# GuidoManni/BodySLAM

Hardware: AMD Instinct MI355X
Metric: frames/sec depth+pose+back-proj, 640x480 seq (higher is better)
Workload: dtype f16

## Files before the change

bodyslam_amd/csrc/upconv_fused.hip:

```cpp
#include "common.h"

namespace bs {

namespace ucf {
constexpr int C = 128, CO = 32, TW = 16, TH = 16, LW = 11, LH = 11, NR = LW * LH;
constexpr int TAB = 2048;
constexpr int PLANE = NR * 128;
constexpr int WROWS = 3 * CO;
constexpr int WPLANE = WROWS * 128;
constexpr int YSTRIDE = 400;
constexpr int YBYTES = NR * YSTRIDE;
template <int MODE> constexpr int a_planes() { return 2 + MODE; }
template <int MODE> constexpr int lds_bytes() { return TAB + a_planes<MODE>() * PLANE + a_planes<MODE>() * WPLANE + YBYTES; }
}

struct UpconvFusedArgs {
    const void* x;
    const void* w;
    const float* bias;
    void* out;
    int B, Hin, Win, Hout, Wout;
    float sy, sx;
    int relu, ntx, nty, ntiles;
    int sa0, sb0, sa1, sb1;
};

template <typename T, int SPLIT, int MODE>
__global__ __launch_bounds__(512) void upconv_fused_kernel(const UpconvFusedArgs p) {
    using namespace ucf;
    typedef typename T16<T>::v8 v8;
    typedef int i32x4_ __attribute__((ext_vector_type(4)));
    typedef int i32x8_ __attribute__((ext_vector_type(8)));
    typedef float f32x2 __attribute__((ext_vector_type(2)));
    constexpr int NPL = a_planes<MODE>();
    constexpr bool FULL = MODE == 2;
    constexpr int ROWB = MODE == 0 ? 2 * C : 4 * C;
    constexpr int OFF_A = TAB, OFF_W = OFF_A + NPL * PLANE, OFF_Y = OFF_W + NPL * WPLANE;
    extern __shared__ __attribute__((aligned(16))) char smem[];
    const int tid = threadIdx.x, lane = tid & 63;
    const int wave = __builtin_amdgcn_readfirstlane(tid >> 6);
    const int frow = lane & 15, fq = lane >> 4;
    const int Hin = p.Hin, Win = p.Win, Hout = p.Hout, Wout = p.Wout;

    auto lo_idx = [&](int r, float s, int n) {
        int i0 = (int)(s * (float)r);
        return i0 > n - 1 ? n - 1 : i0;
    };
    struct Win_ { int b, ty0, tx0, wy0, wx0, LWc, LHc; };
    auto window = [&](int tile) {
        Win_ w;
        const int txi = tile % p.ntx, t2 = tile / p.ntx;
        w.tx0 = txi * TW;
        w.ty0 = (t2 % p.nty) * TH;
        w.b = t2 / p.nty;
        const int rmin = w.ty0 > 0 ? w.ty0 - 1 : 0, rmax = w.ty0 + TH < Hout ? w.ty0 + TH : Hout - 1;
        const int cmin = w.tx0 > 0 ? w.tx0 - 1 : 0, cmax = w.tx0 + TW < Wout ? w.tx0 + TW : Wout - 1;
        w.wy0 = lo_idx(rmin, p.sy, Hin);
        w.wx0 = lo_idx(cmin, p.sx, Win);
        int wy1 = lo_idx(rmax, p.sy, Hin), wx1 = lo_idx(cmax, p.sx, Win);
        wy1 += wy1 < Hin - 1 ? 1 : 0;
        wx1 += wx1 < Win - 1 ? 1 : 0;
        w.LWc = wx1 - w.wx0 + 1;
        w.LHc = wy1 - w.wy0 + 1;
        return w;
    };
    const int r8 = lane >> 3, chunk = (lane & 7) ^ r8;
    auto issue_window = [&](const Win_& w) {
        const int nv = w.LWc * w.LHc;
        const char* xb = reinterpret_cast<const char*>(p.x) + ((int64_t)w.b * Hin * Win) * ROWB;
#pragma unroll
        for (int h = 0; h < 2; ++h) {
            const int rg = wave + 8 * h, row = rg * 8 + r8;
            if (row < NR) {
                const int rw = row < nv ? row : nv - 1;
                const int ly = rw / w.LWc, lx = rw - ly * w.LWc;
                const char* px = xb + ((int64_t)(w.wy0 + ly) * Win + (w.wx0 + lx)) * ROWB + chunk * 16;
#pragma unroll
                for (int pl = 0; pl < NPL; ++pl)
                    glds16(px + pl * 128, smem + OFF_A + pl * PLANE + rg * 1024);
            }
        }
    };
    auto issue_weights = [&](int ky) {
        const char* wb = reinterpret_cast<const char*>(p.w) + (int64_t)(ky * WROWS) * ROWB + chunk * 16;
#pragma unroll
        for (int h = 0; h < 2; ++h) {
            const int rg = wave + 8 * h;
            if (rg < WROWS / 8) {
                const char* pw = wb + (int64_t)(rg * 8 + r8) * ROWB;
#pragma unroll
                for (int pl = 0; pl < NPL; ++pl)
                    glds16(pw + pl * 128, smem + OFF_W + pl * WPLANE + rg * 1024);
            }
        }
    };

    const int g = tid & 7, X = (tid >> 3) & 15, seg = tid >> 7;
    const f32x4 bias4 = *reinterpret_cast<const f32x4*>(p.bias + 4 * g);
    const int sca0 = p.sa0 * 0x01010101, scb0 = p.sb0 * 0x01010101, sca1 = p.sa1 * 0x01010101, scb1 = p.sb1 * 0x01010101;
    const int sw = frow & 7;
    const int koff0 = (fq ^ sw) << 4, koff1 = ((4 + fq) ^ sw) << 4;

    int tile = blockIdx.x;
    if (tile >= p.ntiles) return;
    Win_ cur = window(tile);
    issue_window(cur);
    issue_weights(0);
    for (int it = 0; tile < p.ntiles; tile += gridDim.x, ++it) {
        const int next = tile + gridDim.x;
        i32x4_* tabs = reinterpret_cast<i32x4_*>(smem + (it & 1) * (TAB / 2));
        if (tid < TH + 2 + TW + 2) {
            const bool isrow = tid < TH + 2;
            const int r = isrow ? cur.ty0 - 1 + tid : cur.tx0 - 1 + (tid - (TH + 2));
            const int nout = isrow ? Hout : Wout, nin = isrow ? Hin : Win, w0 = isrow ? cur.wy0 : cur.wx0;
            const float s = isrow ? p.sy : p.sx;
            const int unit = isrow ? cur.LWc * YSTRIDE : YSTRIDE;
            i32x4_ e = {0, 0, 0, 0};
            if (r >= 0 && r < nout) {
                const float f = s * (float)r;
                int i0 = (int)f;
                i0 = i0 > nin - 1 ? nin - 1 : i0;
                const int i1 = i0 + (i0 < nin - 1 ? 1 : 0);
                const float l = f - (float)i0, h = 1.0f - l;
                e = i32x4_{(i0 - w0) * unit, (i1 - w0) * unit, __float_as_int(h), __float_as_int(l)};
            }
            tabs[tid] = e;
        }
        const int mg = wave >> 1, ng = wave & 1;
        v8 af[2][4];
        i32x8_ a8h[2], a8l[2];
        f32x4 acc[4];
#pragma unroll
        for (int yy = 0; yy < 4; ++yy) acc[yy] = bias4;
        i32x4_ ctab[3];
#pragma unroll
        for (int ky = 0; ky < 3; ++ky) {
            if (ky == 1 && next < p.ntiles && !(p.relu & 32)) asm volatile("s_waitcnt vmcnt(%0)" ::"n"(2 * NPL) : "memory");
            else asm volatile("s_waitcnt vmcnt(0)" ::: "memory");
            __syncthreads();
            auto ld8 = [&](const char* base) {
                const i32x4_ lo = *reinterpret_cast<const i32x4_*>(base + koff0);
                const i32x4_ hi = *reinterpret_cast<const i32x4_*>(base + koff1);
                return __builtin_shufflevector(lo, hi, 0, 1, 2, 3, 4, 5, 6, 7);
            };
            if (ky == 0) {
#pragma unroll
                for (int i = 0; i < 2; ++i) {
                    const char* ar = smem + OFF_A + (mg * 32 + i * 16 + frow) * 128;
#pragma unroll
                    for (int kk = 0; kk < 4; ++kk) af[i][kk] = *reinterpret_cast<const v8*>(ar + (kk >> 1) * PLANE + ((kk & 1) ? koff1 : koff0));
                    if constexpr (MODE >= 1) a8h[i] = ld8(ar + 2 * PLANE);
                    if constexpr (FULL) a8l[i] = ld8(ar + 3 * PLANE);
                }
#pragma unroll
                for (int kx = 0; kx < 3; ++kx) ctab[kx] = tabs[TH + 2 + X + kx];
            }
            if (!(p.relu & 8)) {
#pragma unroll
                for (int j = 0; j < 3; ++j) {
                    const char* wr = smem + OFF_W + (ng * 48 + j * 16 + frow) * 128;
                    v8 wf[4];
#pragma unroll
                    for (int kk = 0; kk < 4; ++kk) wf[kk] = *reinterpret_cast<const v8*>(wr + (kk >> 1) * WPLANE + ((kk & 1) ? koff1 : koff0));
                    i32x8_ w8l, w8h;
                    if constexpr (MODE >= 1) w8l = ld8(wr + 2 * WPLANE);
                    if constexpr (FULL) w8h = ld8(wr + 3 * WPLANE);
#pragma unroll
                    for (int i = 0; i < 2; ++i) {
                        f32x4 c = {0.f, 0.f, 0.f, 0.f};
#pragma unroll
                        for (int kk = 0; kk < 4; ++kk) c = T16<T>::mfma16(wf[kk], af[i][kk], c);
                        if constexpr (MODE >= 1) c = __builtin_amdgcn_mfma_scale_f32_16x16x128_f8f6f4(w8l, a8h[i], c, 0, 0, 0, scb0, 0, sca0);
                        if constexpr (FULL) c = __builtin_amdgcn_mfma_scale_f32_16x16x128_f8f6f4(w8h, a8l[i], c, 0, 0, 0, scb1, 0, sca1);
                        const int m = mg * 32 + i * 16 + frow;
                        if (m < NR) *reinterpret_cast<f32x4*>(smem + OFF_Y + m * YSTRIDE + (ng * 48 + j * 16) * 4 + fq * 16) = c;
                    }
                }
            }
            __syncthreads();
            if (ky < 2) {
                if (!(p.relu & 2)) issue_weights(ky + 1);
                if (ky == 0 && next < p.ntiles && !(p.relu & 32)) {
                    const Win_ nw = window(next);
                    issue_window(nw);
                }
            } else if (next < p.ntiles) {
                if (!(p.relu & 2)) issue_weights(0);
            }
            if (!(p.relu & 4)) {
                const char* yb = smem + OFF_Y + g * 16;
                auto rowsum = [&](int roff) {
                    f32x2 u01 = {0.f, 0.f}, u23 = {0.f, 0.f};
#pragma unroll
                    for (int kx = 0; kx < 3; ++kx) {
                        const char* q = yb + roff + kx * (CO * 4);
                        const f32x4 q0 = *reinterpret_cast<const f32x4*>(q + ctab[kx][0]);
                        const f32x4 q1 = *reinterpret_cast<const f32x4*>(q + ctab[kx][1]);
                        const float hx = __int_as_float(ctab[kx][2]), lx = __int_as_float(ctab[kx][3]);
                        const f32x2 h2 = {hx, hx}, l2 = {lx, lx};
                        u01 = __builtin_elementwise_fma(h2, f32x2{q0[0], q0[1]}, u01);
                        u23 = __builtin_elementwise_fma(h2, f32x2{q0[2], q0[3]}, u23);
                        u01 = __builtin_elementwise_fma(l2, f32x2{q1[0], q1[1]}, u01);
                        u23 = __builtin_elementwise_fma(l2, f32x2{q1[2], q1[3]}, u23);
                    }
                    return f32x4{u01[0], u01[1], u23[0], u23[1]};
                };
                int have0 = -1, have1 = -1;
                f32x4 U0 = {0.f, 0.f, 0.f, 0.f}, U1 = U0;
#pragma unroll
                for (int yy = 0; yy < 4; ++yy) {
                    const i32x4_ ry = tabs[4 * seg + yy + ky];
                    const int o0 = __builtin_amdgcn_readfirstlane(ry[0]), o1 = __builtin_amdgcn_readfirstlane(ry[1]);
                    if (o0 != have0) {
                        U0 = (o0 == have1) ? U1 : rowsum(o0);
                        have0 = o0;
                    }
                    if (o1 != have1) {
                        U1 = (o1 == have0) ? U0 : rowsum(o1);
                        have1 = o1;
                    }
                    const float hy = __int_as_float(ry[2]), ly = __int_as_float(ry[3]);
                    const f32x2 h2 = {hy, hy}, l2 = {ly, ly};
                    f32x2 a01 = {acc[yy][0], acc[yy][1]}, a23 = {acc[yy][2], acc[yy][3]};
                    a01 = __builtin_elementwise_fma(h2, f32x2{U0[0], U0[1]}, a01);
                    a23 = __builtin_elementwise_fma(h2, f32x2{U0[2], U0[3]}, a23);
                    a01 = __builtin_elementwise_fma(l2, f32x2{U1[0], U1[1]}, a01);
                    a23 = __builtin_elementwise_fma(l2, f32x2{U1[2], U1[3]}, a23);
                    acc[yy] = f32x4{a01[0], a01[1], a23[0], a23[1]};
                }
            }
        }
        const int ox = cur.tx0 + X;
#pragma unroll
        for (int yy = 0; yy < 4; ++yy) {
            const int oy = cur.ty0 + 4 * seg + yy;
            if (ox >= Wout || oy >= Hout || (p.relu & 16)) continue;
            f32x4 a = acc[yy];
            if (p.relu & 1) {
#pragma unroll
                for (int e = 0; e < 4; ++e) a[e] = fmaxf(a[e], 0.0f);
            }
            const int64_t pix = ((int64_t)cur.b * Hout + oy) * Wout + ox;
            typedef T t4 __attribute__((ext_vector_type(4)));
            t4 hi;
            float rl[4];
#pragma unroll
            for (int e = 0; e < 4; ++e) {
                hi[e] = T16<T>::from_f32(a[e]);
                rl[e] = a[e] - T16<T>::to_f32(hi[e]);
            }
            T* out = reinterpret_cast<T*>(p.out);
            if (SPLIT == 0) {
                *reinterpret_cast<t4*>(out + pix * CO + 4 * g) = hi;
            } else if (SPLIT == 1) {
                t4 lo;
#pragma unroll
                for (int e = 0; e < 4; ++e) lo[e] = T16<T>::from_f32(rl[e]);
                *reinterpret_cast<t4*>(out + pix * 2 * CO + 4 * g) = hi;
                *reinterpret_cast<t4*>(out + pix * 2 * CO + CO + 4 * g) = lo;
            } else {
                T* op = out + pix * 2 * CO;
                *reinterpret_cast<t4*>(op + 4 * g) = hi;
                const float sh = __builtin_ldexpf(1.0f, F8_ACT_HI_EXP), sl = __builtin_ldexpf(1.0f, F8_ACT_LO_EXP);
                char* planes = reinterpret_cast<char*>(op + CO);
                *reinterpret_cast<int*>(planes + 4 * g) = f8_pack4(a[0] * sh, a[1] * sh, a[2] * sh, a[3] * sh);
                *reinterpret_cast<int*>(planes + CO + 4 * g) = f8_pack4(rl[0] * sl, rl[1] * sl, rl[2] * sl, rl[3] * sl);
            }
        }
        if (next < p.ntiles) cur = window(next);
    }
}

template <typename T, int SPLIT, int MODE>
static int launch_upconv_fused(const UpconvFusedArgs& a, hipStream_t st) {
    constexpr int smem = ucf::lds_bytes<MODE>();
    static_assert(smem <= 160 * 1024, "LDS budget");
    static_assert((ucf::TH + 2 + ucf::TW + 2) * 16 <= ucf::TAB / 2, "tables");
    BS_MAX_DYNAMIC_LDS(((const void*)upconv_fused_kernel<T, SPLIT, MODE>), smem);
    const int grid = a.ntiles < cu_count() ? a.ntiles : cu_count();
    hipLaunchKernelGGL((upconv_fused_kernel<T, SPLIT, MODE>), dim3(grid), dim3(512), smem, st, a);
    BS_CHECK_LAUNCH();
    return BS_OK;
}

}

extern "C" int bs_upconv_fused(const void* x, const void* w, const float* bias, void* out, int32_t B, int32_t Hin, int32_t Win, int32_t Cin,
                               int32_t Cout, int32_t Hout, int32_t Wout, int32_t flags, int32_t relu, int32_t mode, int32_t sa0, int32_t sb0,
                               int32_t sa1, int32_t sb1, int32_t dtype, void* stream) {
    using namespace bs;
    if (!initialized()) { set_error("bs_upconv_fused: call bs_init first"); return BS_ERR_NOT_INIT; }
    BS_REQUIRE(x && w && bias && out, "bs_upconv_fused: null operand");
    BS_REQUIRE(B > 0 && Hin >= 2 && Win >= 2, "bs_upconv_fused: empty problem");
    BS_REQUIRE(Cin == ucf::C && Cout == ucf::CO, "bs_upconv_fused: built for %d -> %d channels (got %d -> %d): use bs_gemm + bs_upconv_tapsum", ucf::C,
               ucf::CO, Cin, Cout);
    BS_REQUIRE(Hout == 2 * Hin && Wout == 2 * Win && (flags & 1), "bs_upconv_fused: built for x2 upsampling with align_corners (the 11 x 11 window bound)");
    BS_REQUIRE(dtype == BS_F16 || dtype == BS_BF16, "bs_upconv_fused: dtype must be f16 or bf16");
    BS_REQUIRE(mode >= 0 && mode <= 2, "bs_upconv_fused: mode %d (0 single 16-bit operands, 1 weight-rounding correction, 2 both corrections)", mode);
    BS_REQUIRE((mode == 0) == ((flags & 6) == 0), "bs_upconv_fused: single operands write a single 16-bit output, split operands a split one");
    UpconvFusedArgs a;
    a.x = x; a.w = w; a.bias = bias; a.out = out;
    a.B = B; a.Hin = Hin; a.Win = Win; a.Hout = Hout; a.Wout = Wout;
    a.sy = (float)(Hin - 1) / (float)(Hout - 1);
    a.sx = (float)(Win - 1) / (float)(Wout - 1);
    a.relu = relu;
    a.ntx = cdiv(Wout, ucf::TW);
    a.nty = cdiv(Hout, ucf::TH);
    BS_REQUIRE((int64_t)a.ntx * a.nty * B <= 0x7fffffffll, "bs_upconv_fused: too many tiles");
    a.ntiles = a.ntx * a.nty * B;
    a.sa0 = sa0 & 0xff; a.sb0 = sb0 & 0xff; a.sa1 = sa1 & 0xff; a.sb1 = sb1 & 0xff;
    const int split = (flags & 4) ? 2 : ((flags & 2) ? 1 : 0);
    hipStream_t st = reinterpret_cast<hipStream_t>(stream);
#define BS_UCF(TT)                                                                                                          \
    do {                                                                                                                    \
        if (mode == 0) return launch_upconv_fused<TT, 0, 0>(a, st);                                                         \
        if (mode == 1) {                                                                                                    \
            if (split == 2) return launch_upconv_fused<TT, 2, 1>(a, st);                                                    \
            return launch_upconv_fused<TT, 1, 1>(a, st);                                                                    \
        }                                                                                                                   \
        if (split == 2) return launch_upconv_fused<TT, 2, 2>(a, st);                                                        \
        return launch_upconv_fused<TT, 1, 2>(a, st);                                                                        \
    } while (0)
    if (dtype == BS_F16) BS_UCF(f16);
    BS_UCF(bf16);
#undef BS_UCF
}
```

Baseline: 496.4.

## Add overlapped upconv kernel form pipelining half-channel MFMA with interpolation

Adds a second kernel form that splits the 32 output channels into two 16-channel halves with double-buffered weight and intermediate-product LDS slots. The MFMA tap products for one half are computed while the bilinear interpolation of the other half runs, and the next tile's window load and tables are issued during the last step, so matrix work and the interpolation/LDS phase overlap instead of running in sequence. Stores are widened to 8 channels using DPP quad shuffles. It becomes the default path; the old serial form stays behind a flag bit, and compile-time ablation switches are added.

New measurement: 493.2. Within noise of the previous version (-0.7%).

```diff
diff --git a/bodyslam_amd/csrc/upconv_fused.hip b/bodyslam_amd/csrc/upconv_fused.hip
--- a/bodyslam_amd/csrc/upconv_fused.hip
+++ b/bodyslam_amd/csrc/upconv_fused.hip
@@ -1,5 +1,8 @@
 #include "common.h"
 
+#ifndef UCF_ABL
+#define UCF_ABL 0
+#endif
 namespace bs {
 
 namespace ucf {
@@ -12,6 +15,13 @@
 constexpr int YBYTES = NR * YSTRIDE;
 template <int MODE> constexpr int a_planes() { return 2 + MODE; }
 template <int MODE> constexpr int lds_bytes() { return TAB + a_planes<MODE>() * PLANE + a_planes<MODE>() * WPLANE + YBYTES; }
+constexpr int HCO = CO / 2;
+constexpr int HROWS = 3 * HCO;
+constexpr int HPLANE = HROWS * 128;
+constexpr int HSTRIDE = HROWS * 4 + 16;
+constexpr int HBYTES = NR * HSTRIDE;
+template <int MODE> constexpr int lds_bytes_overlap() { return TAB + a_planes<MODE>() * PLANE + 2 * a_planes<MODE>() * HPLANE + 2 * HBYTES; }
+constexpr int SERIAL_BIT = 64;
 }
 
 struct UpconvFusedArgs {
@@ -25,11 +35,118 @@
     int sa0, sb0, sa1, sb1;
 };
 
+namespace ucf {
+struct Win_ { int b, ty0, tx0, wy0, wx0, LWc, LHc; };
+__device__ __forceinline__ int lo_idx(int r, float s, int n) {
+    int i0 = (int)(s * (float)r);
+    return i0 > n - 1 ? n - 1 : i0;
+}
+__device__ __forceinline__ Win_ window(const UpconvFusedArgs& p, int tile) {
+    Win_ w;
+    const int txi = tile % p.ntx, t2 = tile / p.ntx;
+    w.tx0 = txi * TW;
+    w.ty0 = (t2 % p.nty) * TH;
+    w.b = t2 / p.nty;
+    const int rmin = w.ty0 > 0 ? w.ty0 - 1 : 0, rmax = w.ty0 + TH < p.Hout ? w.ty0 + TH : p.Hout - 1;
+    const int cmin = w.tx0 > 0 ? w.tx0 - 1 : 0, cmax = w.tx0 + TW < p.Wout ? w.tx0 + TW : p.Wout - 1;
+    w.wy0 = lo_idx(rmin, p.sy, p.Hin);
+    w.wx0 = lo_idx(cmin, p.sx, p.Win);
+    int wy1 = lo_idx(rmax, p.sy, p.Hin), wx1 = lo_idx(cmax, p.sx, p.Win);
+    wy1 += wy1 < p.Hin - 1 ? 1 : 0;
+    wx1 += wx1 < p.Win - 1 ? 1 : 0;
+    w.LWc = wx1 - w.wx0 + 1;
+    w.LHc = wy1 - w.wy0 + 1;
+    return w;
+}
+typedef int i32x4_ __attribute__((ext_vector_type(4)));
+__device__ __forceinline__ i32x4_ table_entry(int r, int nout, int nin, int w0, float s, int unit) {
+    i32x4_ e = {0, 0, 0, 0};
+    if (r >= 0 && r < nout) {
+        const float f = s * (float)r;
+        int i0 = (int)f;
+        i0 = i0 > nin - 1 ? nin - 1 : i0;
+        const int i1 = i0 + (i0 < nin - 1 ? 1 : 0);
+        const float l = f - (float)i0, h = 1.0f - l;
+        e = i32x4_{(i0 - w0) * unit, (i1 - w0) * unit, __float_as_int(h), __float_as_int(l)};
+    }
+    return e;
+}
+template <typename T, int SPLIT>
+__device__ __forceinline__ void store4(const UpconvFusedArgs& p, int64_t pix, int c0, f32x4 a) {
+    if (p.relu & 1) {
+#pragma unroll
+        for (int e = 0; e < 4; ++e) a[e] = fmaxf(a[e], 0.0f);
+    }
+    typedef T t4 __attribute__((ext_vector_type(4)));
+    t4 hi;
+    float rl[4];
+#pragma unroll
+    for (int e = 0; e < 4; ++e) {
+        hi[e] = T16<T>::from_f32(a[e]);
+        rl[e] = a[e] - T16<T>::to_f32(hi[e]);
+    }
+    T* out = reinterpret_cast<T*>(p.out);
+    if (SPLIT == 0) {
+        *reinterpret_cast<t4*>(out + pix * CO + c0) = hi;
+    } else if (SPLIT == 1) {
+        t4 lo;
+#pragma unroll
+        for (int e = 0; e < 4; ++e) lo[e] = T16<T>::from_f32(rl[e]);
+        *reinterpret_cast<t4*>(out + pix * 2 * CO + c0) = hi;
+        *reinterpret_cast<t4*>(out + pix * 2 * CO + CO + c0) = lo;
+    } else {
+        T* op = out + pix * 2 * CO;
+        *reinterpret_cast<t4*>(op + c0) = hi;
+        const float sh = __builtin_ldexpf(1.0f, F8_ACT_HI_EXP), sl = __builtin_ldexpf(1.0f, F8_ACT_LO_EXP);
+        char* planes = reinterpret_cast<char*>(op + CO);
+        *reinterpret_cast<int*>(planes + c0) = f8_pack4(a[0] * sh, a[1] * sh, a[2] * sh, a[3] * sh);
+        *reinterpret_cast<int*>(planes + CO + c0) = f8_pack4(rl[0] * sl, rl[1] * sl, rl[2] * sl, rl[3] * sl);
+    }
+}
+template <typename T, int SPLIT>
+__device__ __forceinline__ void store8(const UpconvFusedArgs& p, int64_t pix, int c0, const f32x4& a_lo, const f32x4& a_hi) {
+    float a[8];
+#pragma unroll
+    for (int e = 0; e < 4; ++e) a[e] = a_lo[e], a[4 + e] = a_hi[e];
+    if (p.relu & 1) {
+#pragma unroll
+        for (int e = 0; e < 8; ++e) a[e] = fmaxf(a[e], 0.0f);
+    }
+    typedef T t8 __attribute__((ext_vector_type(8)));
+    typedef int i32x2_ __attribute__((ext_vector_type(2)));
+    t8 hi;
+    float rl[8];
+#pragma unroll
+    for (int e = 0; e < 8; ++e) {
+        hi[e] = T16<T>::from_f32(a[e]);
+        rl[e] = a[e] - T16<T>::to_f32(hi[e]);
+    }
+    T* out = reinterpret_cast<T*>(p.out);
+    if (SPLIT == 0) {
+        *reinterpret_cast<t8*>(out + pix * CO + c0) = hi;
+    } else if (SPLIT == 1) {
+        t8 lo;
+#pragma unroll
+        for (int e = 0; e < 8; ++e) lo[e] = T16<T>::from_f32(rl[e]);
+        *reinterpret_cast<t8*>(out + pix * 2 * CO + c0) = hi;
+        *reinterpret_cast<t8*>(out + pix * 2 * CO + CO + c0) = lo;
+    } else {
+        T* op = out + pix * 2 * CO;
+        *reinterpret_cast<t8*>(op + c0) = hi;
+        const float sh = __builtin_ldexpf(1.0f, F8_ACT_HI_EXP), sl = __builtin_ldexpf(1.0f, F8_ACT_LO_EXP);
+        char* planes = reinterpret_cast<char*>(op + CO);
+        *reinterpret_cast<i32x2_*>(planes + c0) =
+            i32x2_{f8_pack4(a[0] * sh, a[1] * sh, a[2] * sh, a[3] * sh), f8_pack4(a[4] * sh, a[5] * sh, a[6] * sh, a[7] * sh)};
+        *reinterpret_cast<i32x2_*>(planes + CO + c0) =
+            i32x2_{f8_pack4(rl[0] * sl, rl[1] * sl, rl[2] * sl, rl[3] * sl), f8_pack4(rl[4] * sl, rl[5] * sl, rl[6] * sl, rl[7] * sl)};
+    }
+}
+}
+
 template <typename T, int SPLIT, int MODE>
-__global__ __launch_bounds__(512) void upconv_fused_kernel(const UpconvFusedArgs p) {
+__device__ __forceinline__ void upconv_serial(const UpconvFusedArgs& p) {
     using namespace ucf;
     typedef typename T16<T>::v8 v8;
-    typedef int i32x4_ __attribute__((ext_vector_type(4)));
     typedef int i32x8_ __attribute__((ext_vector_type(8)));
     typedef float f32x2 __attribute__((ext_vector_type(2)));
     constexpr int NPL = a_planes<MODE>();
@@ -42,28 +159,7 @@
     const int frow = lane & 15, fq = lane >> 4;
     const int Hin = p.Hin, Win = p.Win, Hout = p.Hout, Wout = p.Wout;
 
-    auto lo_idx = [&](int r, float s, int n) {
-        int i0 = (int)(s * (float)r);
-        return i0 > n - 1 ? n - 1 : i0;
-    };
-    struct Win_ { int b, ty0, tx0, wy0, wx0, LWc, LHc; };
-    auto window = [&](int tile) {
-        Win_ w;
-        const int txi = tile % p.ntx, t2 = tile / p.ntx;
-        w.tx0 = txi * TW;
-        w.ty0 = (t2 % p.nty) * TH;
-        w.b = t2 / p.nty;
-        const int rmin = w.ty0 > 0 ? w.ty0 - 1 : 0, rmax = w.ty0 + TH < Hout ? w.ty0 + TH : Hout - 1;
-        const int cmin = w.tx0 > 0 ? w.tx0 - 1 : 0, cmax = w.tx0 + TW < Wout ? w.tx0 + TW : Wout - 1;
-        w.wy0 = lo_idx(rmin, p.sy, Hin);
-        w.wx0 = lo_idx(cmin, p.sx, Win);
-        int wy1 = lo_idx(rmax, p.sy, Hin), wx1 = lo_idx(cmax, p.sx, Win);
-        wy1 += wy1 < Hin - 1 ? 1 : 0;
-        wx1 += wx1 < Win - 1 ? 1 : 0;
-        w.LWc = wx1 - w.wx0 + 1;
-        w.LHc = wy1 - w.wy0 + 1;
-        return w;
-    };
+    auto window = [&](int tile) { return ucf::window(p, tile); };
     const int r8 = lane >> 3, chunk = (lane & 7) ^ r8;
     auto issue_window = [&](const Win_& w) {
         const int nv = w.LWc * w.LHc;
@@ -115,16 +211,7 @@
             const int nout = isrow ? Hout : Wout, nin = isrow ? Hin : Win, w0 = isrow ? cur.wy0 : cur.wx0;
             const float s = isrow ? p.sy : p.sx;
             const int unit = isrow ? cur.LWc * YSTRIDE : YSTRIDE;
-            i32x4_ e = {0, 0, 0, 0};
-            if (r >= 0 && r < nout) {
-                const float f = s * (float)r;
-                int i0 = (int)f;
-                i0 = i0 > nin - 1 ? nin - 1 : i0;
-                const int i1 = i0 + (i0 < nin - 1 ? 1 : 0);
-                const float l = f - (float)i0, h = 1.0f - l;
-                e = i32x4_{(i0 - w0) * unit, (i1 - w0) * unit, __float_as_int(h), __float_as_int(l)};
-            }
-            tabs[tid] = e;
+            tabs[tid] = table_entry(r, nout, nin, w0, s, unit);
         }
         const int mg = wave >> 1, ng = wave & 1;
         v8 af[2][4];
@@ -235,52 +322,269 @@
         for (int yy = 0; yy < 4; ++yy) {
             const int oy = cur.ty0 + 4 * seg + yy;
             if (ox >= Wout || oy >= Hout || (p.relu & 16)) continue;
-            f32x4 a = acc[yy];
-            if (p.relu & 1) {
-#pragma unroll
-                for (int e = 0; e < 4; ++e) a[e] = fmaxf(a[e], 0.0f);
-            }
-            const int64_t pix = ((int64_t)cur.b * Hout + oy) * Wout + ox;
-            typedef T t4 __attribute__((ext_vector_type(4)));
-            t4 hi;
-            float rl[4];
-#pragma unroll
-            for (int e = 0; e < 4; ++e) {
-                hi[e] = T16<T>::from_f32(a[e]);
-                rl[e] = a[e] - T16<T>::to_f32(hi[e]);
-            }
-            T* out = reinterpret_cast<T*>(p.out);
-            if (SPLIT == 0) {
-                *reinterpret_cast<t4*>(out + pix * CO + 4 * g) = hi;
-            } else if (SPLIT == 1) {
-                t4 lo;
-#pragma unroll
-                for (int e = 0; e < 4; ++e) lo[e] = T16<T>::from_f32(rl[e]);
-                *reinterpret_cast<t4*>(out + pix * 2 * CO + 4 * g) = hi;
-                *reinterpret_cast<t4*>(out + pix * 2 * CO + CO + 4 * g) = lo;
-            } else {
-                T* op = out + pix * 2 * CO;
-                *reinterpret_cast<t4*>(op + 4 * g) = hi;
-                const float sh = __builtin_ldexpf(1.0f, F8_ACT_HI_EXP), sl = __builtin_ldexpf(1.0f, F8_ACT_LO_EXP);
-                char* planes = reinterpret_cast<char*>(op + CO);
-                *reinterpret_cast<int*>(planes + 4 * g) = f8_pack4(a[0] * sh, a[1] * sh, a[2] * sh, a[3] * sh);
-                *reinterpret_cast<int*>(planes + CO + 4 * g) = f8_pack4(rl[0] * sl, rl[1] * sl, rl[2] * sl, rl[3] * sl);
-            }
+            store4<T, SPLIT>(p, ((int64_t)cur.b * Hout + oy) * Wout + ox, 4 * g, acc[yy]);
         }
         if (next < p.ntiles) cur = window(next);
     }
+}
+
+template <typename T, int SPLIT, int MODE>
+__device__ __forceinline__ void upconv_overlap(const UpconvFusedArgs& p) {
+    using namespace ucf;
+    typedef typename T16<T>::v8 v8;
+    typedef int i32x8_ __attribute__((ext_vector_type(8)));
+    typedef float f32x2 __attribute__((ext_vector_type(2)));
+    constexpr int NPL = a_planes<MODE>();
+    constexpr bool FULL = MODE == 2;
+    constexpr int ROWB = MODE == 0 ? 2 * C : 4 * C;
+    constexpr int WSLOT = NPL * HPLANE;
+    constexpr int OFF_A = TAB, OFF_W = OFF_A + NPL * PLANE, OFF_Y = OFF_W + 2 * WSLOT;
+    extern __shared__ __attribute__((aligned(16))) char smem[];
+    const int tid = threadIdx.x, lane = tid & 63;
+    const int wave = __builtin_amdgcn_readfirstlane(tid >> 6);
+    const int frow = lane & 15, fq = lane >> 4;
+    const int Hin = p.Hin, Win = p.Win, Hout = p.Hout, Wout = p.Wout;
+
+    const int r8 = lane >> 3, chunk = (lane & 7) ^ r8;
+    auto issue_window = [&](const Win_& w) {
+        const int nv = w.LWc * w.LHc;
+        const char* xb = reinterpret_cast<const char*>(p.x) + ((int64_t)w.b * Hin * Win) * ROWB;
+#pragma unroll
+        for (int h = 0; h < 2; ++h) {
+            const int rg = wave + 8 * h, row = rg * 8 + r8;
+            if (row < NR) {
+                const int rw = row < nv ? row : nv - 1;
+                const int ly = rw / w.LWc, lx = rw - ly * w.LWc;
+                const char* px = xb + ((int64_t)(w.wy0 + ly) * Win + (w.wx0 + lx)) * ROWB + chunk * 16;
+#pragma unroll
+                for (int pl = 0; pl < NPL; ++pl)
+                    glds16(px + pl * 128, smem + OFF_A + pl * PLANE + rg * 1024);
+            }
+        }
+    };
+    const unsigned wlane = (unsigned)(((wave >> 1) * CO + 8 * (wave & 1) + r8) * ROWB + chunk * 16);
+    auto issue_weights = [&](int s) {
+        if (wave < HROWS / 8) {
+            const int ky = s >> 1, h = s & 1;
+            const char* pw = reinterpret_cast<const char*>(p.w) + (3 * ky * CO + HCO * h) * ROWB + wlane;
+#pragma unroll
+            for (int pl = 0; pl < NPL; ++pl)
+                glds16(pw + pl * 128, smem + OFF_W + h * WSLOT + pl * HPLANE + wave * 1024);
+        }
+    };
+
+    const int g = tid & 3, X = (tid >> 2) & 15;
+    constexpr int OFF_BIAS = (TH + 2 + TW + 2) * 16;
+    const int sca0 = p.sa0 * 0x01010101, scb0 = p.sb0 * 0x01010101, sca1 = p.sa1 * 0x01010101, scb1 = p.sb1 * 0x01010101;
+    const int sw = frow & 7;
+    const int koff0 = (fq ^ sw) << 4, koff1 = ((4 + fq) ^ sw) << 4;
+    const int mg = wave >> 1, ng = wave & 1;
+    const int rowP = (2 * mg + ng) * 16 + frow, rowS = (2 * mg + 1 - ng) * 16 + frow;
+
+    auto ld8 = [&](const char* base) {
+        const i32x4_ lo = *reinterpret_cast<const i32x4_*>(base + koff0);
+        const i32x4_ hi = *reinterpret_cast<const i32x4_*>(base + koff1);
+        return __builtin_shufflevector(lo, hi, 0, 1, 2, 3, 4, 5, 6, 7);
+    };
+    v8 af[2][4];
+    i32x8_ a8h[2], a8l[2];
+    auto load_window = [&]() {
+#pragma unroll
+        for (int i = 0; i < 2; ++i) {
+            const char* ar = smem + OFF_A + (i == 0 ? rowP : rowS) * 128;
+#pragma unroll
+            for (int kk = 0; kk < 4; ++kk) af[i][kk] = *reinterpret_cast<const v8*>(ar + (kk >> 1) * PLANE + ((kk & 1) ? koff1 : koff0));
+            if constexpr (MODE >= 1) a8h[i] = ld8(ar + 2 * PLANE);
+            if constexpr (FULL) a8l[i] = ld8(ar + 3 * PLANE);
+        }
+    };
+    f32x4 c[3];
+    auto products = [&](int slot, int j) {
+        const char* wr = smem + OFF_W + slot * WSLOT + ((j == 0 ? 2 * ng : 1) * 16 + frow) * 128;
+        v8 wf[4];
+#pragma unroll
+        for (int kk = 0; kk < 4; ++kk) wf[kk] = *reinterpret_cast<const v8*>(wr + (kk >> 1) * HPLANE + ((kk & 1) ? koff1 : koff0));
+        i32x8_ w8l, w8h;
+        if constexpr (MODE >= 1) w8l = ld8(wr + 2 * HPLANE);
+        if constexpr (FULL) w8h = ld8(wr + 3 * HPLANE);
+#pragma unroll
+        for (int i = 0; i < 2 - j; ++i) {
+            f32x4 d = {0.f, 0.f, 0.f, 0.f};
+#pragma unroll
+            for (int kk = 0; kk < 4; ++kk) d = T16<T>::mfma16(wf[kk], af[i][kk], d);
+            if constexpr (MODE >= 1) d = __builtin_amdgcn_mfma_scale_f32_16x16x128_f8f6f4(w8l, a8h[i], d, 0, 0, 0, scb0, 0, sca0);
+            if constexpr (FULL) d = __builtin_amdgcn_mfma_scale_f32_16x16x128_f8f6f4(w8h, a8l[i], d, 0, 0, 0, scb1, 0, sca1);
+            c[2 * j + i] = d;
+        }
+    };
+    auto put_products = [&](int buf) {
+        __builtin_amdgcn_sched_barrier(0);
+        asm volatile("s_nop 15\n\ts_nop 15" : "+v"(c[0]), "+v"(c[1]), "+v"(c[2])::"memory");
+        __builtin_amdgcn_sched_barrier(0);
+        char* yw = smem + OFF_Y + buf * HBYTES + fq * 16;
+        if (rowP < NR) {
+            *reinterpret_cast<f32x4*>(yw + rowP * HSTRIDE + 2 * ng * (HCO * 4)) = c[0];
+            *reinterpret_cast<f32x4*>(yw + rowP * HSTRIDE + HCO * 4) = c[2];
+        }
+        if (rowS < NR) *reinterpret_cast<f32x4*>(yw + rowS * HSTRIDE + 2 * ng * (HCO * 4)) = c[1];
+    };
+    auto put_tables = [&](i32x4_* tabs, const Win_& w) {
+        if (tid < TH + 2 + TW + 2) {
+            const bool isrow = tid < TH + 2;
+            const int r = isrow ? w.ty0 - 1 + tid : w.tx0 - 1 + (tid - (TH + 2));
+            tabs[tid] = table_entry(r, isrow ? Hout : Wout, isrow ? Hin : Win, isrow ? w.wy0 : w.wx0, isrow ? p.sy : p.sx,
+                                    isrow ? w.LWc * HSTRIDE : HSTRIDE);
+        }
+    };
+    f32x4 acc[2][2];
+    auto quad = [&](const f32x4& v, int ctrl) {
+        f32x4 r;
+#pragma unroll
+        for (int e = 0; e < 4; ++e) {
+            const int x = __float_as_int(v[e]);
+            r[e] = __int_as_float(ctrl == 0 ? __builtin_amdgcn_update_dpp(x, x, 0x88, 0xf, 0xf, false)
+                                            : __builtin_amdgcn_update_dpp(x, x, 0xdd, 0xf, 0xf, false));
+        }
+        return r;
+    };
+    auto store_tile = [&](const Win_& w) {
+        const int ox = w.tx0 + X;
+#pragma unroll
+        for (int yy = 0; yy < 2; ++yy) {
+            const int oy = w.ty0 + 2 * wave + yy;
+            const f32x4 l0 = quad(acc[0][yy], 0), l1 = quad(acc[1][yy], 0), h0 = quad(acc[0][yy], 1), h1 = quad(acc[1][yy], 1);
+            if (ox >= Wout || oy >= Hout || (UCF_ABL & 16)) continue;
+            store8<T, SPLIT>(p, ((int64_t)w.b * Hout + oy) * Wout + ox, 8 * g, g < 2 ? l0 : l1, g < 2 ? h0 : h1);
+        }
+    };
+
+    const i32x4_* tabs = nullptr;
+    i32x4_ ctab[3];
+    auto rowsum = [&](const char* yb, int roff) {
+        f32x2 u01 = {0.f, 0.f}, u23 = {0.f, 0.f};
+#pragma unroll
+        for (int kx = 0; kx < 3; ++kx) {
+            const char* q = yb + roff + kx * (HCO * 4);
+            const f32x4 q0 = *reinterpret_cast<const f32x4*>(q + ctab[kx][0]);
+            const f32x4 q1 = *reinterpret_cast<const f32x4*>(q + ctab[kx][1]);
+            const float hx = __int_as_float(ctab[kx][2]), lx = __int_as_float(ctab[kx][3]);
+            const f32x2 h2 = {hx, hx}, l2 = {lx, lx};
+            u01 = __builtin_elementwise_fma(h2, f32x2{q0[0], q0[1]}, u01);
+            u23 = __builtin_elementwise_fma(h2, f32x2{q0[2], q0[3]}, u23);
+            u01 = __builtin_elementwise_fma(l2, f32x2{q1[0], q1[1]}, u01);
+            u23 = __builtin_elementwise_fma(l2, f32x2{q1[2], q1[3]}, u23);
+        }
+        return f32x4{u01[0], u01[1], u23[0], u23[1]};
+    };
+    auto rowfma = [&](f32x4& a, const i32x4_& r, const f32x4& U0, const f32x4& U1) {
+        const float hy = __int_as_float(r[2]), ly = __int_as_float(r[3]);
+        const f32x2 h2 = {hy, hy}, l2 = {ly, ly};
+        f32x2 a01 = {a[0], a[1]}, a23 = {a[2], a[3]};
+        a01 = __builtin_elementwise_fma(h2, f32x2{U0[0], U0[1]}, a01);
+        a23 = __builtin_elementwise_fma(h2, f32x2{U0[2], U0[3]}, a23);
+        a01 = __builtin_elementwise_fma(l2, f32x2{U1[0], U1[1]}, a01);
+        a23 = __builtin_elementwise_fma(l2, f32x2{U1[2], U1[3]}, a23);
+        a = f32x4{a01[0], a01[1], a23[0], a23[1]};
+    };
+    i32x4_ ra, rb;
+    f32x4 UA, UB;
+    auto interpolate0 = [&](int ky, int h) {
+        const char* yb = smem + OFF_Y + h * HBYTES + g * 16;
+        ra = tabs[2 * wave + ky];
+        rb = tabs[2 * wave + 1 + ky];
+        UA = rowsum(yb, __builtin_amdgcn_readfirstlane(ra[0]));
+        if constexpr (FULL) __builtin_amdgcn_sched_barrier(0);
+        UB = rowsum(yb, __builtin_amdgcn_readfirstlane(ra[1]));
+    };
+    auto interpolate1 = [&](int h) {
+        const char* yb = smem + OFF_Y + h * HBYTES + g * 16;
+        const int a0 = __builtin_amdgcn_readfirstlane(ra[0]), a1 = __builtin_amdgcn_readfirstlane(ra[1]);
+        const int b0 = __builtin_amdgcn_readfirstlane(rb[0]);
+        const f32x4 UC = rowsum(yb, __builtin_amdgcn_readfirstlane(rb[1]));
+        const f32x4 UD = b0 == a0 ? UA : (b0 == a1 ? UB : UC);
+        rowfma(acc[h][0], ra, UA, UB);
+        rowfma(acc[h][1], rb, UD, UC);
+    };
+
+    int tile = blockIdx.x;
+    if (tile >= p.ntiles) return;
+    Win_ cur = window(p, tile), prev = cur;
+    issue_window(cur);
+    issue_weights(0);
+    issue_weights(1);
+    put_tables(reinterpret_cast<i32x4_*>(smem), cur);
+    if (tid < CO) reinterpret_cast<float*>(smem + OFF_BIAS)[tid] = p.bias[tid];
+    asm volatile("s_waitcnt vmcnt(0)" ::: "memory");
+    __syncthreads();
+    load_window();
+    products(0, 0);
+    products(0, 1);
+    put_products(0);
+    __syncthreads();
+    for (int it = 0;; ++it) {
+        const int next = tile + gridDim.x;
+        const bool has_next = next < p.ntiles;
+        const Win_ nw = window(p, has_next ? next : tile);
+        tabs = reinterpret_cast<const i32x4_*>(smem + (it & 1) * (TAB / 2));
+#pragma unroll 1
+        for (int ky = 0; ky < 3; ++ky) {
+#pragma unroll
+            for (int h = 0; h < 2; ++h) {
+                const int s = 2 * ky + h;
+                if (s == 0) {
+                    if (it > 0) store_tile(prev);
+#pragma unroll
+                    for (int hh = 0; hh < 2; ++hh) acc[hh][0] = acc[hh][1] = *reinterpret_cast<const f32x4*>(smem + OFF_BIAS + (HCO * hh + 4 * g) * 4);
+#pragma unroll
+                    for (int kx = 0; kx < 3; ++kx) ctab[kx] = tabs[TH + 2 + X + kx];
+                }
+                if ((s < 4 || has_next) && !(UCF_ABL & 2)) issue_weights(s < 4 ? s + 2 : s - 4);
+                if (s == 0 && has_next && !(UCF_ABL & 32)) issue_window(nw);
+                if (s == 5 && has_next) {
+                    load_window();
+                    put_tables(reinterpret_cast<i32x4_*>(smem + ((it + 1) & 1) * (TAB / 2)), nw);
+                }
+                if (!(UCF_ABL & 8)) products(1 - h, 0);
+                if (!(UCF_ABL & 4)) interpolate0(ky, h);
+                __builtin_amdgcn_sched_barrier(0);
+                if (!(UCF_ABL & 8)) products(1 - h, 1);
+                if (!(UCF_ABL & 4)) interpolate1(h);
+                if (!(UCF_ABL & 8)) put_products(1 - h);
+                if (s == 0 && has_next && !(UCF_ABL & 32)) asm volatile("s_waitcnt vmcnt(%0)" ::"n"(2 * NPL) : "memory");
+                else asm volatile("s_waitcnt vmcnt(0)" ::: "memory");
+                __syncthreads();
+            }
+        }
+        if (!has_next) break;
+        prev = cur;
+        cur = nw;
+        tile = next;
+    }
+    store_tile(cur);
+}
+
+template <typename T, int SPLIT, int MODE, int FORM>
+__global__ __launch_bounds__(512) void upconv_fused_kernel(const UpconvFusedArgs p) {
+    if constexpr (FORM == 0) upconv_serial<T, SPLIT, MODE>(p);
+    else upconv_overlap<T, SPLIT, MODE>(p);
+}
+
+template <typename T, int SPLIT, int MODE, int FORM>
+static int launch_upconv_form(const UpconvFusedArgs& a, hipStream_t st) {
+    constexpr int smem = FORM == 0 ? ucf::lds_bytes<MODE>() : ucf::lds_bytes_overlap<MODE>();
+    static_assert(smem <= 160 * 1024, "LDS budget");
+    static_assert((ucf::TH + 2 + ucf::TW + 2) * 16 + ucf::CO * 4 <= ucf::TAB / 2, "tables (and, overlapped form, the bias behind the first set)");
+    BS_MAX_DYNAMIC_LDS(((const void*)upconv_fused_kernel<T, SPLIT, MODE, FORM>), smem);
+    const int grid = a.ntiles < cu_count() ? a.ntiles : cu_count();
+    hipLaunchKernelGGL((upconv_fused_kernel<T, SPLIT, MODE, FORM>), dim3(grid), dim3(512), smem, st, a);
+    BS_CHECK_LAUNCH();
+    return BS_OK;
 }
 
 template <typename T, int SPLIT, int MODE>
 static int launch_upconv_fused(const UpconvFusedArgs& a, hipStream_t st) {
-    constexpr int smem = ucf::lds_bytes<MODE>();
-    static_assert(smem <= 160 * 1024, "LDS budget");
-    static_assert((ucf::TH + 2 + ucf::TW + 2) * 16 <= ucf::TAB / 2, "tables");
-    BS_MAX_DYNAMIC_LDS(((const void*)upconv_fused_kernel<T, SPLIT, MODE>), smem);
-    const int grid = a.ntiles < cu_count() ? a.ntiles : cu_count();
-    hipLaunchKernelGGL((upconv_fused_kernel<T, SPLIT, MODE>), dim3(grid), dim3(512), smem, st, a);
-    BS_CHECK_LAUNCH();
-    return BS_OK;
+    if (a.relu & ucf::SERIAL_BIT) return launch_upconv_form<T, SPLIT, MODE, 0>(a, st);
+    return launch_upconv_form<T, SPLIT, MODE, 1>(a, st);
 }
 
 }
```
